# OmarZOS/deep-learning-at-scale

Hardware: AMD Instinct MI355X
Metric: rows/sec (whole node), LSTM seq64 regression at 1/2/4/8 MI355X; val MSE parity (higher is better)
Workload: dtype bf16; 1 GPU; global_batch=8192, per_gpu_batch=8192, seq_len=64, parallelism=dp1

## Files before the change

deep-learning-at-scale_amd/csrc/binding.cpp:

```cpp
#include <torch/extension.h>
#include <ATen/hip/impl/HIPStreamMasqueradingAsCUDA.h>
#include <ATen/hip/impl/HIPGuardImplMasqueradingAsCUDA.h>

#include <cstdlib>
#include <map>
#include <type_traits>
#include <mutex>
#include <vector>

#include "kernels.h"

namespace {

using wf::bf16_t;

int diag_env(const char* name, int dflt) {
  if (wf::dbg_mask() != ~0) return dflt;
  const char* v = std::getenv(name);
  return v != nullptr ? std::atoi(v) : dflt;
}

bool disable_glds() {
  static const bool off = diag_env("WELLFLOW_NO_GLDS", 0) == 1;
  return off;
}

hipStream_t cur_stream() { return c10::hip::getCurrentHIPStreamMasqueradingAsCUDA().stream(); }

void check_t(const at::Tensor& t, at::ScalarType dt, const char* name) {
  TORCH_CHECK(t.defined(), name, ": undefined tensor");
  TORCH_CHECK(t.is_cuda(), name, ": must be a GPU tensor");
  TORCH_CHECK(t.scalar_type() == dt, name, ": expected dtype ", dt, " got ", t.scalar_type());
  TORCH_CHECK(t.is_contiguous(), name, ": must be contiguous");
  TORCH_CHECK(reinterpret_cast<uintptr_t>(t.data_ptr()) % 16 == 0, name,
              ": data pointer must be 16-byte aligned");
}

void check_extent(const at::Tensor& t, int64_t need, const char* name) {
  TORCH_CHECK(t.numel() >= need, name, ": needs at least ", need, " elements, has ", t.numel());
}

bf16_t* bfp(const at::Tensor& t) { return reinterpret_cast<bf16_t*>(t.data_ptr()); }
float* fp(const at::Tensor& t) { return t.data_ptr<float>(); }

template <class T>
T* opt_ptr(const c10::optional<at::Tensor>& t, at::ScalarType dt, const char* name,
           int64_t need) {
  if (!t.has_value() || !t->defined()) return nullptr;
  check_t(*t, dt, name);
  check_extent(*t, need, name);
  return reinterpret_cast<T*>(t->data_ptr());
}

int64_t operand_extent(bool mn, int64_t rows, int64_t K, int64_t ld) {
  if (rows == 0 || K == 0) return 0;
  return mn ? (K - 1) * ld + rows : (rows - 1) * ld + K;
}

void gemm(const at::Tensor& A, bool a_mn, int64_t lda, const at::Tensor& B, bool b_mn, int64_t ldb,
          int64_t M, int64_t N, int64_t K, int64_t ksplit, c10::optional<at::Tensor> outF,
          c10::optional<at::Tensor> outH, int64_t ldo, c10::optional<at::Tensor> bias,
          c10::optional<at::Tensor> mask, int64_t ldm, double mask_scale,
          c10::optional<at::Tensor> colsum, double alpha, double beta, int64_t act, bool atomic,
          double drop_p, int64_t seed, int64_t big_tile, c10::optional<at::Tensor> seed_dev) {
  TORCH_CHECK(wf::dw_tile_valid(big_tile), "gemm: tile ", big_tile, " does not exist; valid ids are 0 (128x128), ",
              "1 (256x128), 3 (256x192), 4 / 5 (256x192, 5- / 4-slot ring), 7 (best for N)");
  check_t(A, at::kBFloat16, "A");
  check_t(B, at::kBFloat16, "B");
  TORCH_CHECK(M > 0 && N > 0 && K > 0, "gemm: empty problem");
  TORCH_CHECK(lda % 8 == 0 && ldb % 8 == 0, "gemm: lda/ldb must be multiples of 8");
  TORCH_CHECK(a_mn ? (M % 8 == 0) : (K % 8 == 0), "gemm: A contiguous extent must be a multiple of 8");
  TORCH_CHECK(b_mn ? (N % 8 == 0) : (K % 8 == 0), "gemm: B contiguous extent must be a multiple of 8");
  TORCH_CHECK(a_mn ? lda >= M : lda >= K, "gemm: lda too small");
  TORCH_CHECK(b_mn ? ldb >= N : ldb >= K, "gemm: ldb too small");
  check_extent(A, operand_extent(a_mn, M, K, lda), "A");
  check_extent(B, operand_extent(b_mn, N, K, ldb), "B");
  TORCH_CHECK(ldo >= N, "gemm: ldo < N");
  const int64_t out_need = (M - 1) * ldo + N;
  wf::GemmEpilogue e;
  e.outF = opt_ptr<float>(outF, at::kFloat, "outF", out_need);
  e.outH = opt_ptr<bf16_t>(outH, at::kBFloat16, "outH", out_need);
  TORCH_CHECK(e.outF || e.outH, "gemm: need an output");
  TORCH_CHECK(!atomic || (e.outF && !e.outH && beta == 0.0), "gemm: atomic needs outF only, beta 0");
  TORCH_CHECK(beta == 0.0 || e.outF, "gemm: beta needs outF");
  e.ldo = ldo;
  e.bias = opt_ptr<float>(bias, at::kFloat, "bias", N);
  if (mask.has_value() && mask->defined()) TORCH_CHECK(ldm >= N, "gemm: ldm < N");
  e.mask = opt_ptr<bf16_t>(mask, at::kBFloat16, "mask", (M - 1) * ldm + N);
  e.ldm = ldm;
  e.mask_scale = (float)mask_scale;
  e.colsum = opt_ptr<float>(colsum, at::kFloat, "colsum", N);
  e.alpha = (float)alpha;
  e.beta = (float)beta;
  e.act = (int)act;
  e.atomic = atomic ? 1 : 0;
  e.drop_p = (float)drop_p;
  e.seed = (unsigned long long)seed;
  if (seed_dev.has_value() && seed_dev->defined()) {
    TORCH_CHECK(seed_dev->is_cuda() && seed_dev->scalar_type() == at::kLong && seed_dev->numel() >= 1,
                "gemm: seed_dev must be a GPU int64 tensor");
    e.seed_dev = reinterpret_cast<const long long*>(seed_dev->data_ptr<int64_t>());
  }
  e.big_tile = (int)big_tile;
  TORCH_CHECK(ksplit == 1 || atomic, "gemm: split-K needs atomic accumulation");
  e.stage_ok = (e.outH != nullptr && e.outF == nullptr && !atomic && beta == 0.0 && N % 8 == 0 &&
                ldo % 8 == 0 && (e.mask == nullptr || ldm % 8 == 0))
                   ? 1 : 0;
  const int64_t Mc = (M + 127) / 128 * 128, Nc = (N + 127) / 128 * 128;
  int64_t kchunk = (K + std::max<int64_t>(ksplit, 1) - 1) / std::max<int64_t>(ksplit, 1);
  kchunk = (kchunk + 63) / 64 * 64;
  const bool glds_ok = (K % 64 == 0) && (kchunk % 64 == 0) &&
                       A.numel() >= operand_extent(a_mn, Mc, K, lda) + (a_mn ? 0 : 0) &&
                       B.numel() >= operand_extent(b_mn, Nc, K, ldb) &&
                       (a_mn || Mc == M || lda >= K) && (b_mn || Nc == N || ldb >= K);
  const c10::hip::OptionalHIPGuardMasqueradingAsCUDA guard(A.device());
  wf::launch_gemm(bfp(A), lda, a_mn, bfp(B), ldb, b_mn, (int)M, (int)N, (int)K, (int)ksplit, e,
                  cur_stream(), glds_ok && !disable_glds());
}

wf::LstmDims lstm_dims(int64_t B, int64_t T, int64_t F, int64_t KX, int64_t H) {
  TORCH_CHECK(B > 0 && T > 0 && H > 0, "lstm: bad dims");
  TORCH_CHECK(H % 128 == 0, "lstm: hidden size must be a multiple of 128");
  TORCH_CHECK(KX % 64 == 0 && F + 1 <= KX, "lstm: KX must be a multiple of 64 and > F");
  wf::LstmDims d;
  d.B = (int)B; d.T = (int)T; d.F = (int)F; d.KX = (int)KX; d.H = (int)H;
  d.xcd_map = diag_env("WELLFLOW_XCD_MAP", 1) == 0 ? 0 : 1;
  d.nt = diag_env("WELLFLOW_NT", 1) == 0 ? 0 : 1;
  const char* pd = std::getenv("WELLFLOW_PF_DBG");
  d.dbg = (pd != nullptr ? std::atoi(pd) : 0) & wf::dbg_mask();
  const char* sl = std::getenv("WELLFLOW_SPIN_LIMIT");
  d.spin_limit = sl != nullptr ? (unsigned)std::strtoul(sl, nullptr, 10) : 0u;
  const char* ft = std::getenv("WELLFLOW_FORCE_TIMEOUT");
  if (ft != nullptr && ft[0] == '1') d.dbg |= 1 << 21;
  return d;
}

void check_lstm_state(const at::Tensor& XH, const at::Tensor& Cst, const at::Tensor& S,
                      const wf::LstmDims& d) {
  const int64_t KA = d.KX + d.H, G = 4 * d.H;
  const int64_t Bp = (d.B + 15) / 16 * 16;
  check_t(XH, at::kBFloat16, "XH");
  check_t(Cst, at::kBFloat16, "Cst");
  check_t(S, at::kBFloat16, "S");
  check_extent(XH, (int64_t)(d.T + 1) * d.B * KA, "XH");
  check_extent(Cst, (int64_t)(d.T + 1) * Bp * d.H, "Cst");
  check_extent(S, (int64_t)d.T * Bp * G, "S");
}

void lstm_pack_x(const at::Tensor& x, const at::Tensor& XH, int64_t B, int64_t T, int64_t F,
                 int64_t KX, int64_t H, bool full) {
  auto d = lstm_dims(B, T, F, KX, H);
  check_t(x, at::kFloat, "x");
  check_extent(x, B * T * F, "x");
  check_t(XH, at::kBFloat16, "XH");
  check_extent(XH, (T + 1) * B * (KX + H), "XH");
  const c10::hip::OptionalHIPGuardMasqueradingAsCUDA guard(x.device());
  wf::launch_lstm_pack_x(fp(x), bfp(XH), d, cur_stream(), full);
}

void lstm_pack_x_win(const at::Tensor& table, const at::Tensor& starts, const at::Tensor& idx, const at::Tensor& XH,
                     int64_t B, int64_t T, int64_t F, int64_t KX, int64_t H, bool full) {
  auto d = lstm_dims(B, T, F, KX, H);
  check_t(table, at::kFloat, "table");
  TORCH_CHECK(table.dim() == 2 && table.size(1) == F && table.size(0) >= T, "lstm_pack_x_win: table must be [>= T][F]");
  check_t(starts, at::kLong, "starts");
  check_t(idx, at::kLong, "idx");
  check_extent(idx, B, "idx");
  TORCH_CHECK(starts.numel() >= 1, "lstm_pack_x_win: no windows");
  check_t(XH, at::kBFloat16, "XH");
  check_extent(XH, (T + 1) * B * (KX + H), "XH");
  const c10::hip::OptionalHIPGuardMasqueradingAsCUDA guard(table.device());
  wf::launch_lstm_pack_x(fp(table), bfp(XH), d, cur_stream(), full, reinterpret_cast<const long*>(starts.data_ptr<int64_t>()),
                         reinterpret_cast<const long*>(idx.data_ptr<int64_t>()), starts.numel(), table.size(0));
}

void lstm_forward(const at::Tensor& XH, const at::Tensor& Wp, const at::Tensor& Cst,
                  const at::Tensor& S, const at::Tensor& cf32, int64_t B, int64_t T, int64_t F, int64_t KX,
                  int64_t H, int64_t variant) {
  auto d = lstm_dims(B, T, F, KX, H);
  d.fwd_variant = (int)variant;
  check_lstm_state(XH, Cst, S, d);
  check_t(Wp, at::kBFloat16, "Wp");
  check_extent(Wp, 4 * H * (KX + H), "Wp");
  check_t(cf32, at::kFloat, "cf32");
  check_extent(cf32, (B + 15) / 16 * 16 * H, "cf32");
  const c10::hip::OptionalHIPGuardMasqueradingAsCUDA guard(XH.device());
  auto s = cur_stream();
  for (int t = 0; t < d.T; ++t) wf::launch_lstm_fwd_step(t, bfp(XH), bfp(Wp), bfp(Cst), bfp(S), fp(cf32), d, s);
}

void check_sync(const at::Tensor& sync) {
  check_t(sync, at::kInt, "sync");
}

bool persistent_status(int st, const char* what) {
  TORCH_CHECK(st >= 0, what, ": launch failed: ", hipGetErrorString((hipError_t)(-st)));
  return st == 1;
}

bool lstm_forward_persistent(const at::Tensor& XH, const at::Tensor& Wp, const at::Tensor& Cst,
                             const at::Tensor& S, const at::Tensor& sync, int64_t B, int64_t T, int64_t F,
                             int64_t KX, int64_t H) {
  auto d = lstm_dims(B, T, F, KX, H);
  check_lstm_state(XH, Cst, S, d);
  check_t(Wp, at::kBFloat16, "Wp");
  check_extent(Wp, 4 * H * (KX + H), "Wp");
  check_sync(sync);
  const c10::hip::OptionalHIPGuardMasqueradingAsCUDA guard(XH.device());
  return persistent_status(wf::launch_lstm_fwd_persistent(bfp(XH), bfp(Wp), bfp(Cst), bfp(S),
                                                          reinterpret_cast<unsigned*>(sync.data_ptr<int>()),
                                                          sync.numel(), d, cur_stream()),
                           "persistent LSTM forward");
}

void check_lstm_bwd(const at::Tensor& WhhT, const at::Tensor& DG, const at::Tensor& dcarry, const at::Tensor& dy,
                    const at::Tensor& w_out, int64_t B, int64_t T, int64_t H) {
  check_t(WhhT, at::kBFloat16, "WhhT");
  check_extent(WhhT, H * 4 * H, "WhhT");
// ... 1178 lines not shown
```

deep-learning-at-scale_amd/csrc/gemm.hip:

```cpp
#include <cstdlib>

#include "gemm_core.h"
#include "kernels.h"

namespace wf {

__device__ __forceinline__ unsigned long long drop_seed(const GemmEpilogue& e) {
  return e.seed_dev != nullptr ? e.seed ^ ((unsigned long long)e.seed_dev[0] * 0xD1B54A32D192ED03ull) : e.seed;
}

template <int BM, int BN, int LA, int LB, int STAGES, int WM = 2, int WN = 2>
__global__ __launch_bounds__(64 * WM * WN) void gemm_kernel(const bf16_t* __restrict__ A, long lda,
                                                   const bf16_t* __restrict__ B, long ldb,
                                                   int M, int N, int K, int kchunk,
                                                   GemmEpilogue e) {
  using C = GemmCfg<BM, BN, LA, LB, WM, WN>;
  constexpr int LDSB = STAGES * C::STAGE > C::LDS_BYTES ? STAGES * C::STAGE : C::LDS_BYTES;
  __shared__ __attribute__((aligned(16))) char smem[LDSB];
  const int tiles_n = (N + BN - 1) / BN;
  const int tiles = ((M + BM - 1) / BM) * tiles_n;
  const int L = xcd_remap(blockIdx.x, gridDim.x);
  const int split = L / tiles, t = L % tiles;
  const int m0 = (t / tiles_n) * BM, n0 = (t % tiles_n) * BN;
  const int kbeg = split * kchunk;
// ... 23 lines not shown
        *reinterpret_cast<uint4*>(mt + chunk_off(row, c8)) = v;
      }
      __syncthreads();
    }
#pragma unroll
    for (int j = 0; j < C::TN; ++j) {
      const int n = cc.col(j);
      const int col = n - n0;
      const bool nok = n < N;
      const float bn = (e.bias != nullptr && nok) ? e.bias[n] : 0.f;
      float csum = 0.f;
#pragma unroll
      for (int i = 0; i < C::TM; ++i) {
#pragma unroll
        for (int r = 0; r < 4; ++r) {
          const int m = cc.row(i, r);
          const int row = m - m0;
          const int lo = chunk_off(row, col >> 3) + (col & 7);
          float v = e.alpha * acc[i][j][r] + bn;
          if (e.act == 1) v = fmaxf(v, 0.f);
          if (e.drop_p > 0.f)
            v = uniform_hash(drop_seed(e), (unsigned long long)m * N + n) >= e.drop_p
                    ? v * (1.f / (1.f - e.drop_p)) : 0.f;
          if (e.mask != nullptr) v = bf2f(mt[lo]) > 0.f ? v * e.mask_scale : 0.f;
          const bf16_t vb = f2bf(v);
          ot[lo] = vb;
          if (nok && m < M) csum += bf2f(vb);
        }
      }
      if (e.colsum != nullptr) {
        csum += __shfl_xor(csum, 16, 64);
        csum += __shfl_xor(csum, 32, 64);
        if ((threadIdx.x & 63) < 16 && nok) atomicAdd(e.colsum + n, csum);
      }
    }
    __syncthreads();
    for (int q = threadIdx.x; q < BM * CPR; q += C::NT) {
      const int row = q / CPR, c8 = q % CPR;
      const int m = m0 + row, n = n0 + c8 * 8;
      if (m < M && n < N)
        *reinterpret_cast<uint4*>(e.outH + (size_t)m * e.ldo + n) =
            *reinterpret_cast<const uint4*>(ot + chunk_off(row, c8));
    }
    return;
  }

#pragma unroll
  for (int j = 0; j < C::TN; ++j) {
    const int n = cc.col(j);
    const bool nok = n < N;
    const float bn = (e.bias != nullptr && nok) ? e.bias[n] : 0.f;
    float csum = 0.f;
#pragma unroll
    for (int i = 0; i < C::TM; ++i) {
#pragma unroll
      for (int r = 0; r < 4; ++r) {
        const int m = cc.row(i, r);
        if (!nok || m >= M) continue;
        float v = e.alpha * acc[i][j][r];
        const size_t o = (size_t)m * e.ldo + n;
        if (e.atomic) {
          atomicAdd(e.outF + o, v);
          continue;
        }
        if (e.beta != 0.f) v += e.beta * e.outF[o];
        v += bn;
        if (e.act == 1) v = fmaxf(v, 0.f);
        if (e.drop_p > 0.f)
          v = uniform_hash(drop_seed(e), (unsigned long long)m * N + n) >= e.drop_p
                  ? v * (1.f / (1.f - e.drop_p)) : 0.f;
        if (e.mask != nullptr)
          v = bf2f(e.mask[(size_t)m * e.ldm + n]) > 0.f ? v * e.mask_scale : 0.f;
        csum += v;
        if (e.outF != nullptr) e.outF[o] = v;
        if (e.outH != nullptr) e.outH[o] = f2bf(v);
      }
    }
    if (e.colsum != nullptr) {
      csum += __shfl_xor(csum, 16, 64);
      csum += __shfl_xor(csum, 32, 64);
      if ((threadIdx.x & 63) < 16 && nok) atomicAdd(e.colsum + n, csum);
    }
  }
}

template <int BM, int BN, int LA, int LB>
static void launch_cfg(const bf16_t* A, long lda, const bf16_t* B, long ldb, int M, int N, int K,
                       int ksplit, const GemmEpilogue& e, hipStream_t s, bool glds_ok) {
  const int tiles = ((M + BM - 1) / BM) * ((N + BN - 1) / BN);
  if (ksplit < 1) ksplit = 1;
  int kchunk = (K + ksplit - 1) / ksplit;
  kchunk = (kchunk + 63) / 64 * 64;
  if (kchunk < 64) kchunk = 64;
  const int nsplit = (K + kchunk - 1) / kchunk;
  const dim3 grid(tiles * (nsplit > 0 ? nsplit : 1));
  if (glds_ok && K % 64 == 0)
    hipLaunchKernelGGL((gemm_kernel<BM, BN, LA, LB, 3>), grid, dim3(256), 0, s, A, lda, B, ldb, M,
                       N, K, kchunk, e);
  else
    hipLaunchKernelGGL((gemm_kernel<BM, BN, LA, LB, 0>), grid, dim3(256), 0, s, A, lda, B, ldb, M,
                       N, K, kchunk, e);
}


static void launch_dw_big(const bf16_t* A, long lda, const bf16_t* B, long ldb, int M, int N, int K,
                          int ksplit, const GemmEpilogue& e, hipStream_t s) {
  constexpr int BM = 256, BN = 128;
  const int tiles = ((M + BM - 1) / BM) * ((N + BN - 1) / BN);
  int kchunk = ((K + ksplit - 1) / ksplit + 63) / 64 * 64;
  const int nsplit = (K + kchunk - 1) / kchunk;
  hipLaunchKernelGGL((gemm_kernel<BM, BN, MN_CONTIG, MN_CONTIG, 3, 4, 2>), dim3(tiles * nsplit),
                     dim3(512), 0, s, A, lda, B, ldb, M, N, K, kchunk, e);
}

template <int BM, int BN, int STAGES, int WM, int WN, int PRIO = 0>
__global__ __launch_bounds__(64 * WM * WN) void gemm_dw_kernel(const bf16_t* __restrict__ A, long lda,
                                                      const bf16_t* __restrict__ B, long ldb, int N,
                                                      int kchunk, int tiles, float* __restrict__ out,
                                                      long ldo, float alpha) {
  using C = GemmCfg<BM, BN, MN_CONTIG, MN_CONTIG, WM, WN>;
  __shared__ __attribute__((aligned(16))) char smem[STAGES * C::STAGE];
  const int tiles_n = N / BN;
  const int L = xcd_remap(blockIdx.x, gridDim.x);
  const int split = L / tiles, t = L % tiles;
  const int m0 = (t / tiles_n) * BM, n0 = (t % tiles_n) * BN;
  f32x4 acc[C::TM][C::TN];
  gemm_mainloop_glds2<C, STAGES, PRIO>(A, lda, B, ldb, split * kchunk, kchunk / 64, m0, n0, smem, acc);
  const AccCoord<C> cc(m0, n0);
#pragma unroll
  for (int j = 0; j < C::TN; ++j)
#pragma unroll
    for (int i = 0; i < C::TM; ++i)
#pragma unroll
      for (int r = 0; r < 4; ++r)
        atomicAdd(out + (size_t)cc.row(i, r) * ldo + cc.col(j), alpha * acc[i][j][r]);
}

static int equal_ksplit(int K, int ksplit) {
  int nsplit = ksplit;
  while (nsplit > 1 && K % (64 * nsplit) != 0) --nsplit;
  return nsplit;
}

static void launch_dw_192(const bf16_t* A, long lda, const bf16_t* B, long ldb, int M, int N, int K,
                          int ksplit, const GemmEpilogue& e, hipStream_t s) {
  constexpr int BM = 256, BN = 192;
  const int tiles = (M / BM) * (N / BN);
  const int nsplit = equal_ksplit(K, ksplit);
  const int kchunk = K / nsplit;
  hipLaunchKernelGGL((gemm_dw_kernel<BM, BN, 2, 4, 2, 1>), dim3(tiles * nsplit), dim3(512), 0, s, A, lda, B, ldb,
                     N, kchunk, tiles, e.outF, e.ldo, e.alpha);
}

template <int BM, int BN, int NSLOT, int WM, int WN, int PRIO, int BKD = 32>
__global__ __launch_bounds__(64 * WM * WN) void gemm_dw_h_kernel(const bf16_t* __restrict__ A, long lda,
                                                        const bf16_t* __restrict__ B, long ldb, int N,
                                                        int kchunk, int tiles, float* __restrict__ out,
                                                        long ldo, float alpha, float* __restrict__ slab,
                                                        long slab_stride) {
  using C = GemmCfg<BM, BN, MN_CONTIG, MN_CONTIG, WM, WN>;
  constexpr int STAGE = (BM + BN) * BKD * 2;
  __shared__ __attribute__((aligned(16))) char smem[NSLOT * STAGE];
  const int tiles_n = N / BN;
  const int L = xcd_remap(blockIdx.x, gridDim.x);
  const int split = L / tiles, t = L % tiles;
  const int m0 = (t / tiles_n) * BM, n0 = (t % tiles_n) * BN;
  f32x4 acc[C::TM][C::TN];
  gemm_mainloop_glds_h<C, NSLOT, PRIO, BKD>(A, lda, B, ldb, split * kchunk, kchunk / BKD, m0, n0, smem, acc);
  const AccCoord<C> cc(m0, n0);
  if (slab != nullptr) {
    float* o = slab + (size_t)split * slab_stride;
#pragma unroll
    for (int j = 0; j < C::TN; ++j)
#pragma unroll
      for (int i = 0; i < C::TM; ++i)
#pragma unroll
        for (int r = 0; r < 4; ++r) o[(size_t)cc.row(i, r) * ldo + cc.col(j)] = alpha * acc[i][j][r];
    return;
  }
#pragma unroll
  for (int j = 0; j < C::TN; ++j)
#pragma unroll
    for (int i = 0; i < C::TM; ++i)
#pragma unroll
      for (int r = 0; r < 4; ++r)
        atomicAdd(out + (size_t)cc.row(i, r) * ldo + cc.col(j), alpha * acc[i][j][r]);
}

static void launch_dw_192h(const bf16_t* A, long lda, const bf16_t* B, long ldb, int M, int N, int K,
                           int ksplit, int nslot, const GemmEpilogue& e, hipStream_t s) {
  constexpr int BM = 256, BN = 192;
  const int tiles = (M / BM) * (N / BN);
  const int nsplit = equal_ksplit(K, ksplit);
  const int kchunk = K / nsplit;
  const dim3 grid(tiles * nsplit);
  if (nslot == 5)
    hipLaunchKernelGGL((gemm_dw_h_kernel<BM, BN, 5, 4, 2, 1>), grid, dim3(512), 0, s, A, lda, B, ldb, N, kchunk,
                       tiles, e.outF, e.ldo, e.alpha, nullptr, 0L);
  else
    hipLaunchKernelGGL((gemm_dw_h_kernel<BM, BN, 4, 4, 2, 1>), grid, dim3(512), 0, s, A, lda, B, ldb, N, kchunk,
                       tiles, e.outF, e.ldo, e.alpha, nullptr, 0L);
}

__global__ __launch_bounds__(256) void dw_slab_reduce_kernel(float* __restrict__ out, const float* __restrict__ slab,
                                                             int nsplit, long n4) {
  const long i = (long)blockIdx.x * 256 + threadIdx.x;
  if (i >= n4) return;
  const float4* src = reinterpret_cast<const float4*>(slab) + i;
  float4 a = reinterpret_cast<float4*>(out)[i];
  for (int s0 = 0; s0 < nsplit; s0 += 8) {
    float4 v[8];
#pragma unroll
    for (int j = 0; j < 8; ++j) v[j] = s0 + j < nsplit ? src[(size_t)(s0 + j) * n4] : make_float4(0.f, 0.f, 0.f, 0.f);
#pragma unroll
    for (int j = 0; j < 8; ++j) {
      a.x += v[j].x;
      a.y += v[j].y;
      a.z += v[j].z;
      a.w += v[j].w;
    }
  }
  reinterpret_cast<float4*>(out)[i] = a;
}

static void launch_dw_288w(const bf16_t* A, long lda, const bf16_t* B, long ldb, int M, int N, int K,
                           int ksplit, const GemmEpilogue& e, hipStream_t s) {
  constexpr int BM = 256, BN = 288;
  const int tiles = (M / BM) * (N / BN);
  static const int cus = [] {
    int dev = 0, n = 0;
    if (hipGetDevice(&dev) != hipSuccess || hipDeviceGetAttribute(&n, hipDeviceAttributeMultiprocessorCount, dev) != hipSuccess)
      return 256;
    return n;
  }();
  if (ksplit * tiles > cus && cus / tiles >= 1) ksplit = cus / tiles;
  const int nsplit = equal_ksplit(K, ksplit);
  const int kchunk = K / nsplit;
  const long mn = (long)M * N;
  const bool use_slab = e.slab != nullptr && e.ldo == N && nsplit > 1 && (long)nsplit * mn <= e.slab_cap && mn % 4 == 0;
  hipLaunchKernelGGL((gemm_dw_h_kernel<BM, BN, 4, 4, 2, 1, 32>), dim3(tiles * nsplit), dim3(512), 0, s, A, lda, B,
                     ldb, N, kchunk, tiles, e.outF, e.ldo, e.alpha, use_slab ? e.slab : nullptr, use_slab ? mn : 0L);
  if (use_slab) {
    const long n4 = mn / 4;
    hipLaunchKernelGGL(dw_slab_reduce_kernel, dim3((unsigned)((n4 + 255) / 256)), dim3(256), 0, s, e.outF,
                       (const float*)e.slab, nsplit, n4);
  }
}

void launch_gemm(const bf16_t* A, long lda, int a_mn, const bf16_t* B, long ldb, int b_mn, int M,
                 int N, int K, int ksplit, const GemmEpilogue& e, hipStream_t s, bool glds_ok) {
  if (a_mn && b_mn && glds_ok && e.atomic && e.big_tile != kDwGeneric && M % 256 == 0 && K % 64 == 0) {
    const int ks = ksplit < 1 ? 1 : ksplit;
    if (e.big_tile == kDwBest && N % 288 == 0)
      launch_dw_288w(A, lda, B, ldb, M, N, K, ks, e, s);
    else if ((e.big_tile == kDw256x192Ring5 || e.big_tile == kDw256x192Ring4) && N % 192 == 0)
      launch_dw_192h(A, lda, B, ldb, M, N, K, ks, e.big_tile == kDw256x192Ring5 ? 5 : 4, e, s);
    else if (e.big_tile != kDw256x128 && N % 192 == 0)
      launch_dw_192(A, lda, B, ldb, M, N, K, ks, e, s);
    else
      launch_dw_big(A, lda, B, ldb, M, N, K, ks, e, s);
    return;
  }
  if (!a_mn && !b_mn)
    launch_cfg<128, 128, K_CONTIG, K_CONTIG>(A, lda, B, ldb, M, N, K, ksplit, e, s, glds_ok);
  else if (!a_mn && b_mn)
    launch_cfg<128, 128, K_CONTIG, MN_CONTIG>(A, lda, B, ldb, M, N, K, ksplit, e, s, glds_ok);
  else if (a_mn && !b_mn)
    launch_cfg<128, 128, MN_CONTIG, K_CONTIG>(A, lda, B, ldb, M, N, K, ksplit, e, s, glds_ok);
  else
    launch_cfg<128, 128, MN_CONTIG, MN_CONTIG>(A, lda, B, ldb, M, N, K, ksplit, e, s, glds_ok);
}

}
```

deep-learning-at-scale_amd/csrc/gemm_core.h:

```cpp
#pragma once
#include <type_traits>

#include "common.h"

namespace wf {

enum : int { K_CONTIG = 0, MN_CONTIG = 1 };

typedef __attribute__((address_space(3))) bf16x4 lds_bf16x4;

template <int R>
struct MnSwz {
  static constexpr int C = R / 16;
  static constexpr bool POW2 = (C & (C - 1)) == 0;
  static constexpr int RSH = C == 12 ? 1 : (C == 18 ? 2 : 0);
  __host__ __device__ static constexpr int hmask() { return POW2 ? C - 1 : 7; }
  __device__ static __forceinline__ int hk(int k) { return ((k & 3) | ((k >> 1) & 4)) & hmask(); }
  __device__ static __forceinline__ int pos(int j, int h) { return POW2 ? (j ^ h) : (j + (h >> RSH)) % C; }
  __device__ static __forceinline__ int data(int p, int h) { return POW2 ? (p ^ h) : (p + C - (h >> RSH)) % C; }
};

template <int R, int L, int NT_ = 256>
struct OpTile {
  static constexpr int NT = NT_;
// ... 248 lines not shown
      const int hk = (q | ((g & 1) << 2)) & MnSwz<R>::hmask();
#pragma unroll
      for (int i = 0; i < NB; ++i)
        fb[i] = (8 * g + q) * (R * 2) + (MnSwz<R>::pos((rw >> 4) + i, hk) << 5) + p * 8;
    }
  }

  template <int KK, int TOFF>
  __device__ __forceinline__ bf16x8 frag(const char* smem, int i) const {
    if constexpr (L == K_CONTIG) {
      return *reinterpret_cast<const bf16x8*>(smem + fb[KK] + TOFF + i * 16 * 128);
    } else {
      bf16x8 out;
#pragma unroll
      for (int h = 0; h < 2; ++h) {
        const char* a = smem + fb[i] + TOFF + (KK * 32 + 4 * h) * (R * 2);
        bf16x4 v = __builtin_amdgcn_ds_read_tr16_b64_v4i16((lds_bf16x4*)a);
        out[4 * h + 0] = v[0];
        out[4 * h + 1] = v[1];
        out[4 * h + 2] = v[2];
        out[4 * h + 3] = v[3];
      }
      return out;
    }
  }
};

template <class C, int STAGES, int PRIO = 0>
__device__ __forceinline__ void gemm_mainloop_glds2(const bf16_t* __restrict__ A, long lda,
                                                    const bf16_t* __restrict__ B, long ldb, int kbeg,
                                                    int nk, int m0, int n0, char* smem,
                                                    f32x4 (&acc)[C::TM][C::TN]) {
  static_assert(STAGES >= 2 && STAGES <= 6, "2..6 stages");
  using OA = GldsOperand<C::BM, C::LA_, C::NT>;
  using OB = GldsOperand<C::BN, C::LB_, C::NT>;
  constexpr int STAGE = OA::TILE_BYTES + OB::TILE_BYTES;
  constexpr int LPT = OA::Q::PER_WAVE + OB::Q::PER_WAVE;
  const int lane = threadIdx.x & 63;
  const int wid = __builtin_amdgcn_readfirstlane(threadIdx.x >> 6);
  const int wm = wid / C::WN, wn = wid % C::WN;
#pragma unroll
  for (int i = 0; i < C::TM; ++i)
#pragma unroll
    for (int j = 0; j < C::TN; ++j) acc[i][j] = f32x4{0.f, 0.f, 0.f, 0.f};
  if (nk <= 0) return;
  OA oa;
  OB ob;
  oa.init(A, lda, m0, kbeg, wid, lane);
  ob.init(B, ldb, n0, kbeg, wid, lane);
  FragReader<C::BM, C::LA_, C::WTM> fa;
  FragReader<C::BN, C::LB_, C::WTN> fbr;
  fa.init(wm * C::WTM, lane);
  fbr.init(wn * C::WTN, lane);

#pragma unroll
  for (int s = 0; s < STAGES - 1; ++s) {
    if (s < nk) {
      oa.issue(s, smem + s * STAGE, wid);
      ob.issue(s, smem + s * STAGE + OA::TILE_BYTES, wid);
    }
  }

  auto body = [&](int tt, auto uc) {
    constexpr int u = decltype(uc)::value;
    const int ahead = min(nk - 1, tt + STAGES - 2) - tt;
    if constexpr (STAGES >= 5) {
      if (ahead >= STAGES - 2) wait_vmcnt<(STAGES - 2) * LPT>();
      else if (ahead == 3) wait_vmcnt<3 * LPT>();
      else if (ahead == 2) wait_vmcnt<2 * LPT>();
      else if (ahead == 1) wait_vmcnt<LPT>();
      else wait_vmcnt<0>();
    } else if constexpr (STAGES >= 4) {
      if (ahead >= 2) wait_vmcnt<2 * LPT>();
      else if (ahead == 1) wait_vmcnt<LPT>();
      else wait_vmcnt<0>();
    } else if constexpr (STAGES == 3) {
      if (ahead >= 1) wait_vmcnt<LPT>();
      else wait_vmcnt<0>();
    } else {
      wait_vmcnt<0>();
    }
    __builtin_amdgcn_s_barrier();
    asm volatile("" ::: "memory");
    const int tn = tt + STAGES - 1;
    if (tn < nk) {
      constexpr int sn = (u + STAGES - 1) % STAGES;
      oa.issue(tn, smem + sn * STAGE, wid);
      ob.issue(tn, smem + sn * STAGE + OA::TILE_BYTES, wid);
    }
    static_for<0, 2>([&](auto kc) {
      constexpr int KK = decltype(kc)::value;
      bf16x8 a[C::TM], b[C::TN];
#pragma unroll
      for (int i = 0; i < C::TM; ++i) a[i] = fa.template frag<KK, u * STAGE>(smem, i);
#pragma unroll
      for (int j = 0; j < C::TN; ++j) b[j] = fbr.template frag<KK, u * STAGE + OA::TILE_BYTES>(smem, j);
      if constexpr (PRIO == 1) __builtin_amdgcn_s_setprio(1);
#pragma unroll
      for (int i = 0; i < C::TM; ++i)
#pragma unroll
        for (int j = 0; j < C::TN; ++j)
          acc[i][j] = __builtin_amdgcn_mfma_f32_16x16x32_bf16(a[i], b[j], acc[i][j], 0, 0, 0);
      if constexpr (PRIO == 1) __builtin_amdgcn_s_setprio(0);
    });
  };

  int t = 0;
  for (; t + STAGES <= nk; t += STAGES)
    static_for<0, STAGES>([&](auto uc) { body(t + decltype(uc)::value, uc); });
  static_for<0, STAGES>([&](auto uc) {
    if (t + decltype(uc)::value < nk) body(t + decltype(uc)::value, uc);
  });
  __builtin_amdgcn_s_barrier();
  asm volatile("" ::: "memory");
}

template <int R, int L, int NT, int BKD>
struct GldsOpH {
  static_assert(L == MN_CONTIG, "half-step ring: MN-contiguous operands only");
  static constexpr int BYTES = R * BKD * 2;
  static constexpr int PIECES = BYTES / 1024;
  static constexpr int NW = NT / 64;
  static constexpr int MAXPW = (PIECES + NW - 1) / NW;
  static constexpr int REM = PIECES % NW;
  static_assert(BYTES % 1024 == 0 && PIECES >= NW, "tile image must be whole 1-KiB pieces, >= 1 per wave");
  using SW = MnSwz<R>;
  unsigned src[MAXPW];
  __amdgpu_buffer_rsrc_t rsrc;
  int kstep_bytes;

  __device__ __forceinline__ void init(const bf16_t* p, long ld, int row0, int kbeg, int wid, int lane) {
#pragma unroll
    for (int i = 0; i < MAXPW; ++i) {
      const int o = (i * NW + wid) * 1024 + lane * 16;
      const int k = o / (R * 2), b = o % (R * 2);
      const int col = (SW::data(b >> 5, SW::hk(k)) << 4) + (((b >> 4) & 1) << 3);
      src[i] = (unsigned)(((long)k * ld + col) * 2);
    }
    rsrc = __builtin_amdgcn_make_buffer_rsrc(const_cast<bf16_t*>(p + (size_t)kbeg * ld + row0), 0, 0x7FFFFFFF,
                                             0x00020000);
    kstep_bytes = (int)(BKD * ld * 2);
  }
  __device__ __forceinline__ void issue(int step, char* lds_tile, int wid) const {
    const int so = step * kstep_bytes;
#pragma unroll
    for (int i = 0; i < MAXPW; ++i) {
      if (i + 1 < MAXPW || REM == 0 || wid < REM)
        __builtin_amdgcn_raw_ptr_buffer_load_lds(rsrc, (lds_void*)(lds_tile + (i * NW + wid) * 1024), 16, (int)src[i],
                                                 so, 0, 0);
    }
  }
};

template <class C, int NSLOT, int PRIO = 0, int BKD = 32>
__device__ __forceinline__ void gemm_mainloop_glds_h(const bf16_t* __restrict__ A, long lda,
                                                     const bf16_t* __restrict__ B, long ldb, int kbeg,
                                                     int nh, int m0, int n0, char* smem,
                                                     f32x4 (&acc)[C::TM][C::TN]) {
  static_assert(BKD == 32 || BKD == 64, "32- or 64-deep steps");
  static_assert(NSLOT >= 2 && NSLOT <= 6, "2..6 slots");
  using OA = GldsOpH<C::BM, C::LA_, C::NT, BKD>;
  using OB = GldsOpH<C::BN, C::LB_, C::NT, BKD>;
  static_assert(OA::REM == 0 || OB::REM == 0, "at most one operand with an uneven piece split");
  constexpr int STAGE = OA::BYTES + OB::BYTES;
  constexpr int LHI = OA::MAXPW + OB::MAXPW;
  constexpr int LLO = LHI - ((OA::REM | OB::REM) != 0 ? 1 : 0);
  constexpr int NHI = OA::REM ? OA::REM : (OB::REM ? OB::REM : C::NT / 64);
  const int lane = threadIdx.x & 63;
  const int wid = __builtin_amdgcn_readfirstlane(threadIdx.x >> 6);
  const int wm = wid / C::WN, wn = wid % C::WN;
  const bool hi = wid < NHI;
#pragma unroll
  for (int i = 0; i < C::TM; ++i)
#pragma unroll
    for (int j = 0; j < C::TN; ++j) acc[i][j] = f32x4{0.f, 0.f, 0.f, 0.f};
  if (nh <= 0) return;
  OA oa;
  OB ob;
  oa.init(A, lda, m0, kbeg, wid, lane);
  ob.init(B, ldb, n0, kbeg, wid, lane);
  FragReader<C::BM, C::LA_, C::WTM> fa;
  FragReader<C::BN, C::LB_, C::WTN> fbr;
  fa.init(wm * C::WTM, lane);
  fbr.init(wn * C::WTN, lane);

#pragma unroll
  for (int s = 0; s < NSLOT - 1; ++s) {
    if (s < nh) {
      oa.issue(s, smem + s * STAGE, wid);
      ob.issue(s, smem + s * STAGE + OA::BYTES, wid);
    }
  }
  auto body = [&](int tt, auto uc) {
    constexpr int u = decltype(uc)::value;
    const int ahead = min(nh - 1, tt + NSLOT - 2) - tt;
    __builtin_amdgcn_sched_barrier(0);
    static_for<0, NSLOT - 1>([&](auto ac) {
      constexpr int a = NSLOT - 2 - decltype(ac)::value;
      if (ahead == a) {
        if (hi) wait_vmcnt<a * LHI>();
        else wait_vmcnt<a * LLO>();
      }
    });
    __builtin_amdgcn_s_barrier();
    asm volatile("" ::: "memory");
    const int tn = tt + NSLOT - 1;
    if (tn < nh) {
      constexpr int sn = (u + NSLOT - 1) % NSLOT;
      oa.issue(tn, smem + sn * STAGE, wid);
      ob.issue(tn, smem + sn * STAGE + OA::BYTES, wid);
    }
    int so = u * STAGE;
    asm volatile("" : "+v"(so));
    const char* sl = smem + so;
    static_for<0, BKD / 32>([&](auto kc) {
      constexpr int KK = decltype(kc)::value;
      bf16x8 a[C::TM], b[C::TN];
#pragma unroll
      for (int i = 0; i < C::TM; ++i) a[i] = fa.template frag<KK, 0>(sl, i);
#pragma unroll
      for (int j = 0; j < C::TN; ++j) b[j] = fbr.template frag<KK, OA::BYTES>(sl, j);
      if constexpr (PRIO == 1) __builtin_amdgcn_s_setprio(1);
#pragma unroll
      for (int i = 0; i < C::TM; ++i)
#pragma unroll
        for (int j = 0; j < C::TN; ++j)
          acc[i][j] = __builtin_amdgcn_mfma_f32_16x16x32_bf16(a[i], b[j], acc[i][j], 0, 0, 0);
      if constexpr (PRIO == 1) __builtin_amdgcn_s_setprio(0);
    });
  };
  int t = 0;
  for (; t + NSLOT <= nh; t += NSLOT)
    static_for<0, NSLOT>([&](auto uc) { body(t + decltype(uc)::value, uc); });
  static_for<0, NSLOT>([&](auto uc) {
    if (t + decltype(uc)::value < nh) body(t + decltype(uc)::value, uc);
  });
  __builtin_amdgcn_s_barrier();
  asm volatile("" ::: "memory");
}

template <class C>
struct AccCoord {
  int mb, nb;
  __device__ __forceinline__ AccCoord(int m0, int n0) {
    const int wid = threadIdx.x >> 6;
    mb = m0 + (wid / C::WN) * C::WTM;
    nb = n0 + (wid % C::WN) * C::WTN;
  }
  __device__ __forceinline__ int row(int i, int r) const {
    return mb + i * 16 + 4 * ((threadIdx.x & 63) >> 4) + r;
  }
  __device__ __forceinline__ int col(int j) const { return nb + j * 16 + (threadIdx.x & 15); }
};

}
```

deep-learning-at-scale_amd/csrc/kernels.h:

```cpp
#pragma once
#include <hip/hip_runtime.h>
#include <stdint.h>

namespace wf {

typedef unsigned short bf16_t;

enum DwTile : int {
  kDwGeneric = 0,
  kDw256x128 = 1,
  kDw256x192 = 3,
  kDw256x192Ring5 = 4,
  kDw256x192Ring4 = 5,
  kDwBest = 7,
};
inline bool dw_tile_valid(long t) {
  return t == kDwGeneric || t == kDw256x128 || t == kDw256x192 || t == kDw256x192Ring5 || t == kDw256x192Ring4 ||
         t == kDwBest;
}

struct GemmEpilogue {
  float* outF = nullptr;
  bf16_t* outH = nullptr;
  long ldo = 0;
  const float* bias = nullptr;
  const bf16_t* mask = nullptr;
  long ldm = 0;
  float mask_scale = 1.f;
  float* colsum = nullptr;
  float alpha = 1.f, beta = 0.f;
  int act = 0;
  int atomic = 0;
  float drop_p = 0.f;
  unsigned long long seed = 0;
  const long long* seed_dev = nullptr;
  int stage_ok = 0;
  int big_tile = kDwGeneric;
  float* slab = nullptr;
  long slab_cap = 0;
};

void launch_gemm(const bf16_t* A, long lda, int a_mn, const bf16_t* B, long ldb, int b_mn, int M,
                 int N, int K, int ksplit, const GemmEpilogue& e, hipStream_t s,
                 bool glds_ok = false);

struct LstmDims {
  int B, T, F, KX, H;
  int fwd_variant = 0;
  int bwd_variant = 0;
  int xcd_map = 1;
  int nt = 1;
  int dbg = 0;
  int row_off = 0;
  unsigned spin_limit = 0;
};
int dbg_mask();
void launch_lstm_pack_x(const float* x, bf16_t* XH, LstmDims d, hipStream_t s, bool full = true,
                        const long* starts = nullptr, const long* idx = nullptr, long nwin = 0, long nrows = 0);
void launch_lstm_fwd_step(int t, bf16_t* XH, const bf16_t* Wp, bf16_t* Cst, bf16_t* S, float* cf32,
                          LstmDims d, hipStream_t s);
int lstm_persistent_sync_words(int row_blocks);
long lstm_persistent_sync_total(int row_blocks);
int launch_lstm_fwd_persistent(bf16_t* XH, const bf16_t* Wp, bf16_t* Cst, bf16_t* S, unsigned* sync,
                                long sync_words, LstmDims d, hipStream_t s);
int launch_lstm_bwd_persistent(const bf16_t* WhhT, const bf16_t* Cst, const bf16_t* S, bf16_t* DG,
                                const float* dcarry, unsigned* sync, long sync_words, LstmDims d,
                                hipStream_t s);
void launch_lstm_bwd_step(int t, const bf16_t* WhhT, const bf16_t* Cst, const bf16_t* S,
                          bf16_t* DG, float* dcarry, const float* dy, const float* w_out,
                          LstmDims d, hipStream_t s);
void launch_lstm_pack_weights(const float* W, bf16_t* Wp, bf16_t* WhhT, LstmDims d,
                              hipStream_t s);

bool launch_mlp2_fwd(const bf16_t* X, int Fp, const bf16_t* W1, const float* b1, const bf16_t* W2, const float* b2,
                     const float* w3, const float* b3, const float* y, bf16_t* H1, bf16_t* H2, unsigned* M2,
                     float* dw3, float* db3, float* pred, float* dy, float* loss_sum, float dy_scale, int B,
                     const long long* rows, long nrows, hipStream_t s, float* red = nullptr);
bool launch_mlp2_bwd(const bf16_t* H1, const bf16_t* H2, const unsigned* M2, const float* dy, const float* w3, const bf16_t* W2,
                     const bf16_t* X, int Fp, bf16_t* dZ1, bf16_t* dZ2, float* dW1, float* db1, float* db2,
                     float* dw3, float* db3, int B, const bf16_t* W1, const float* b1, const long long* rows,
                     long nrows, hipStream_t s, float* red = nullptr);
bool launch_mlp2_dw2(const bf16_t* dZ2, const bf16_t* X, int Fp, const long long* rows, long nrows, const bf16_t* W1,
                     const float* b1, int B, int nsplit, float* dW2, hipStream_t s, float* red = nullptr);
constexpr int kMlpRedCopies = 64, kMlpRedCopies2 = 4, kMlpRedRow = 9216;
constexpr int kMlpRedLoss = 0, kMlpRedDb3 = 1, kMlpRedDw3 = 2, kMlpRedDb1 = 258, kMlpRedDb2 = 514, kMlpRedDW1 = 770;
constexpr int kMlpRedSlabRows = 256, kMlpRedSlabRow = 256 * 64;
constexpr long kMlpRedSlabOff = (long)kMlpRedCopies * kMlpRedRow + (long)kMlpRedCopies2 * 65536;
constexpr int kMlpRedSlab2Rows = 256;
constexpr long kMlpRedSlab2Off = kMlpRedSlabOff + (long)kMlpRedSlabRows * kMlpRedSlabRow;
constexpr long kMlpRedFloats = kMlpRedSlab2Off + (long)kMlpRedSlab2Rows * 65536;
int mlp2_train_grid(int B);
constexpr int kMlpSmallScratch = 49728 + 65536;
struct MlpSmallArgs {
  const bf16_t* X;
  const float* Y;
  const long long* rows;
  long nrows;
  int Fp, B, K;
  float* p;
  float* m;
  float* v;
  float* step;
  float lr, b1, b2, eps, wd, dy_scale, clip;
  bf16_t* shadow;
  bf16_t* w2t;
  float* loss_acc;
  float* scr;
  unsigned* sync;
  unsigned spin_limit;
  long oW1, ob1, oW2, ob2, ow3, ob3;
  unsigned long long* stamps;
};
bool launch_mlp_small(const MlpSmallArgs& a, hipStream_t s);
constexpr int kCnnSmallScratch = 2 * 28 * 64 * 16 * 2 + 2 * 64 * 16 * 2;
struct CnnSmallArgs {
  const float* X;
  const float* Y;
  const long long* rows;
  long nrows;
  int B, K, O, taps, filters, drop, loss_kind;
  float keep_scale, clip, scale;
  unsigned seed;
  long long* rng;
  float* p;
  float* vel;
  float* step;
  float lr, decay, momentum, gscale;
  int nesterov;
  float* loss_acc;
  float* scr;
  unsigned* sync;
  unsigned spin_limit;
  unsigned long long* stamps;
};
bool launch_cnn_small(const CnnSmallArgs& a, hipStream_t s);
bool mlp_bwd8();
void launch_mlp2_reduce(float* red, int Fp, int B, float* loss_sum, float* db3, float* dw3, float* db1, float* db2,
                        float* dW1, float* dW2, hipStream_t s, int dw2_rows = 0);
bool launch_mlp2_step(const bf16_t* X, int Fp, const bf16_t* W1, const float* b1, const bf16_t* W2, const float* b2,
                      const float* w3, const float* b3, const float* y, float dy_scale, int B, const long long* rows,
                      long nrows, bf16_t* dZ2, float* pred, float* red, bool dz_frag, hipStream_t s,
                      const bf16_t* W2T = nullptr, float clip = 0.f);
int launch_mlp2_dw2f(const bf16_t* dZ2F, const bf16_t* X, int Fp, const long long* rows, long nrows, const bf16_t* W1,
                     const float* b1, int B, int nsplit, float* red, hipStream_t s);

struct CnnDims {
  int L, C, taps, T, Fp, Kc, O;
  float drop_p;
};
bool cnn_fused_supported(const CnnDims& d);
int cnn_fwd_grid(int B);
int cnn_bwd_chunks(int B);
long cnn_part_floats(int B, const CnnDims& d, long* wd, long* wc, long* f);
void launch_cnn_sgd_pack(float* p, float* g, float* vel, long n, float* step, float lr, float decay, float momentum,
                         int nesterov, float gscale, int zero_g, const CnnDims& d, bf16_t* WcA, bf16_t* WdF,
                         bf16_t* WdB, hipStream_t s, const float* clip = nullptr, float clipvalue = 0.f);
void launch_cnn_pack(const float* Wc, const float* Wd, const CnnDims& d, bf16_t* WcA, bf16_t* WdF, bf16_t* WdB,
                     hipStream_t s);
void launch_cnn_forward(const float* x, int B, const CnnDims& d, const bf16_t* WcA, const bf16_t* WdF,
                        const float* bd, const float* y, float* dout, float* pred, float* part, int train,
                        int loss_kind, float clip, float scale, unsigned seed, const long long* rng, hipStream_t s);
void launch_cnn_backward(const float* x, int B, const CnnDims& d, const bf16_t* WcA, const bf16_t* WdB,
                         const float* dout, unsigned seed, const long long* rng, float* part_wd, float* part_wc,
                         hipStream_t s);
void launch_cnn_reduce(const float* part_wd, const float* part_wc, const float* part_f, int B, const CnnDims& d,
                       float* gWc, float* gWd, float* gbd, float* loss_sum, long long* rng, hipStream_t s);

void launch_head_fwd(const bf16_t* Hm, long ldh, int B, int Hd, const float* w, const float* b0,
                     const float* target, float* pred, float* dy, float* loss_sum, float dy_scale,
                     hipStream_t s);
bool launch_head_fwd_bwd(const bf16_t* Hm, long ldh, int B, int Hd, const float* w, const float* b0,
                         const float* target, float* pred, float* dy, float* loss_sum, float dy_scale, float* dw,
// ... 71 lines not shown
```

Before: 2.020 million rows/s.

## Alternate global-to-LDS load issue between wave halves in 288-wide dW GEMM

Adds a SCHED=1 mode to the GLDS mainloop. Each 4-slot pipeline stage is now loaded by only half of the waves, with the two halves alternating by stage parity, instead of every wave issuing a share of every stage. The aim is to spread memory issue and vmcnt waits so each wave spends less time stalled on loads between MFMA bursts, at the cost of more loads per issuing wave. The 288-wide weight-gradient launcher uses this mode by default, and a WF_DIAG-gated tile id keeps the old schedule available for comparison.

```diff
diff --git a/deep-learning-at-scale_amd/csrc/binding.cpp b/deep-learning-at-scale_amd/csrc/binding.cpp
--- a/deep-learning-at-scale_amd/csrc/binding.cpp
+++ b/deep-learning-at-scale_amd/csrc/binding.cpp
@@ -63,7 +63,7 @@
           c10::optional<at::Tensor> mask, int64_t ldm, double mask_scale,
           c10::optional<at::Tensor> colsum, double alpha, double beta, int64_t act, bool atomic,
           double drop_p, int64_t seed, int64_t big_tile, c10::optional<at::Tensor> seed_dev) {
-  TORCH_CHECK(wf::dw_tile_valid(big_tile), "gemm: tile ", big_tile, " does not exist; valid ids are 0 (128x128), ",
+  TORCH_CHECK(wf::dw_tile_valid(big_tile) || wf::dw_tile_diag(big_tile), "gemm: tile ", big_tile, " does not exist; valid ids are 0 (128x128), ",
               "1 (256x128), 3 (256x192), 4 / 5 (256x192, 5- / 4-slot ring), 7 (best for N)");
   check_t(A, at::kBFloat16, "A");
   check_t(B, at::kBFloat16, "B");
diff --git a/deep-learning-at-scale_amd/csrc/gemm.hip b/deep-learning-at-scale_amd/csrc/gemm.hip
--- a/deep-learning-at-scale_amd/csrc/gemm.hip
+++ b/deep-learning-at-scale_amd/csrc/gemm.hip
@@ -199,7 +199,7 @@
                      N, kchunk, tiles, e.outF, e.ldo, e.alpha);
 }
 
-template <int BM, int BN, int NSLOT, int WM, int WN, int PRIO, int BKD = 32>
+template <int BM, int BN, int NSLOT, int WM, int WN, int PRIO, int BKD = 32, int SCHED = 0>
 __global__ __launch_bounds__(64 * WM * WN) void gemm_dw_h_kernel(const bf16_t* __restrict__ A, long lda,
                                                         const bf16_t* __restrict__ B, long ldb, int N,
                                                         int kchunk, int tiles, float* __restrict__ out,
@@ -213,7 +213,7 @@
   const int split = L / tiles, t = L % tiles;
   const int m0 = (t / tiles_n) * BM, n0 = (t % tiles_n) * BN;
   f32x4 acc[C::TM][C::TN];
-  gemm_mainloop_glds_h<C, NSLOT, PRIO, BKD>(A, lda, B, ldb, split * kchunk, kchunk / BKD, m0, n0, smem, acc);
+  gemm_mainloop_glds_h<C, NSLOT, PRIO, BKD, SCHED>(A, lda, B, ldb, split * kchunk, kchunk / BKD, m0, n0, smem, acc);
   const AccCoord<C> cc(m0, n0);
   if (slab != nullptr) {
     float* o = slab + (size_t)split * slab_stride;
@@ -268,6 +268,17 @@
     }
   }
   reinterpret_cast<float4*>(out)[i] = a;
+}
+
+constexpr int kDw288Sched = 1;
+
+bool dw_tile_diag(long t) {
+#ifdef WF_DIAG
+  return t == kDwDiagSched0;
+#else
+  (void)t;
+  return false;
+#endif
 }
 
 static void launch_dw_288w(const bf16_t* A, long lda, const bf16_t* B, long ldb, int M, int N, int K,
@@ -285,8 +296,16 @@
   const int kchunk = K / nsplit;
   const long mn = (long)M * N;
   const bool use_slab = e.slab != nullptr && e.ldo == N && nsplit > 1 && (long)nsplit * mn <= e.slab_cap && mn % 4 == 0;
-  hipLaunchKernelGGL((gemm_dw_h_kernel<BM, BN, 4, 4, 2, 1, 32>), dim3(tiles * nsplit), dim3(512), 0, s, A, lda, B,
-                     ldb, N, kchunk, tiles, e.outF, e.ldo, e.alpha, use_slab ? e.slab : nullptr, use_slab ? mn : 0L);
+  auto go = [&](auto sc) {
+    hipLaunchKernelGGL((gemm_dw_h_kernel<BM, BN, 4, 4, 2, 1, 32, decltype(sc)::value>), dim3(tiles * nsplit),
+                       dim3(512), 0, s, A, lda, B, ldb, N, kchunk, tiles, e.outF, e.ldo, e.alpha,
+                       use_slab ? e.slab : nullptr, use_slab ? mn : 0L);
+  };
+#ifdef WF_DIAG
+  if (e.big_tile == kDwDiagSched0) go(std::integral_constant<int, 0>{});
+  else
+#endif
+    go(std::integral_constant<int, kDw288Sched>{});
   if (use_slab) {
     const long n4 = mn / 4;
     hipLaunchKernelGGL(dw_slab_reduce_kernel, dim3((unsigned)((n4 + 255) / 256)), dim3(256), 0, s, e.outF,
@@ -298,7 +317,7 @@
                  int N, int K, int ksplit, const GemmEpilogue& e, hipStream_t s, bool glds_ok) {
   if (a_mn && b_mn && glds_ok && e.atomic && e.big_tile != kDwGeneric && M % 256 == 0 && K % 64 == 0) {
     const int ks = ksplit < 1 ? 1 : ksplit;
-    if (e.big_tile == kDwBest && N % 288 == 0)
+    if ((e.big_tile == kDwBest || dw_tile_diag(e.big_tile)) && N % 288 == 0)
       launch_dw_288w(A, lda, B, ldb, M, N, K, ks, e, s);
     else if ((e.big_tile == kDw256x192Ring5 || e.big_tile == kDw256x192Ring4) && N % 192 == 0)
       launch_dw_192h(A, lda, B, ldb, M, N, K, ks, e.big_tile == kDw256x192Ring5 ? 5 : 4, e, s);
diff --git a/deep-learning-at-scale_amd/csrc/gemm_core.h b/deep-learning-at-scale_amd/csrc/gemm_core.h
--- a/deep-learning-at-scale_amd/csrc/gemm_core.h
+++ b/deep-learning-at-scale_amd/csrc/gemm_core.h
@@ -424,24 +424,30 @@
   }
 };
 
-template <class C, int NSLOT, int PRIO = 0, int BKD = 32>
+template <class C, int NSLOT, int PRIO = 0, int BKD = 32, int SCHED = 0>
 __device__ __forceinline__ void gemm_mainloop_glds_h(const bf16_t* __restrict__ A, long lda,
                                                      const bf16_t* __restrict__ B, long ldb, int kbeg,
                                                      int nh, int m0, int n0, char* smem,
                                                      f32x4 (&acc)[C::TM][C::TN]) {
   static_assert(BKD == 32 || BKD == 64, "32- or 64-deep steps");
   static_assert(NSLOT >= 2 && NSLOT <= 6, "2..6 slots");
-  using OA = GldsOpH<C::BM, C::LA_, C::NT, BKD>;
-  using OB = GldsOpH<C::BN, C::LB_, C::NT, BKD>;
+  static_assert(SCHED == 0 || (SCHED == 1 && NSLOT == 4), "alternating issuer: 4 slots (issuer = half step & 1)");
+  constexpr bool ALT = SCHED == 1;
+  constexpr int NWV = C::NT / 64;
+  constexpr int NIW = ALT ? NWV / 2 : NWV;
+  using OA = GldsOpH<C::BM, C::LA_, NIW * 64, BKD>;
+  using OB = GldsOpH<C::BN, C::LB_, NIW * 64, BKD>;
   static_assert(OA::REM == 0 || OB::REM == 0, "at most one operand with an uneven piece split");
   constexpr int STAGE = OA::BYTES + OB::BYTES;
   constexpr int LHI = OA::MAXPW + OB::MAXPW;
   constexpr int LLO = LHI - ((OA::REM | OB::REM) != 0 ? 1 : 0);
-  constexpr int NHI = OA::REM ? OA::REM : (OB::REM ? OB::REM : C::NT / 64);
+  constexpr int NHI = OA::REM ? OA::REM : (OB::REM ? OB::REM : NIW);
   const int lane = threadIdx.x & 63;
   const int wid = __builtin_amdgcn_readfirstlane(threadIdx.x >> 6);
   const int wm = wid / C::WN, wn = wid % C::WN;
-  const bool hi = wid < NHI;
+  const int grp = wid / NIW;
+  const int wq = ALT ? wid % NIW : wid;
+  const bool hi = wq < NHI;
 #pragma unroll
   for (int i = 0; i < C::TM; ++i)
 #pragma unroll
@@ -449,8 +455,8 @@
   if (nh <= 0) return;
   OA oa;
   OB ob;
-  oa.init(A, lda, m0, kbeg, wid, lane);
-  ob.init(B, ldb, n0, kbeg, wid, lane);
+  oa.init(A, lda, m0, kbeg, wq, lane);
+  ob.init(B, ldb, n0, kbeg, wq, lane);
   FragReader<C::BM, C::LA_, C::WTM> fa;
   FragReader<C::BN, C::LB_, C::WTN> fbr;
   fa.init(wm * C::WTM, lane);
@@ -458,29 +464,49 @@
 
 #pragma unroll
   for (int s = 0; s < NSLOT - 1; ++s) {
-    if (s < nh) {
-      oa.issue(s, smem + s * STAGE, wid);
-      ob.issue(s, smem + s * STAGE + OA::BYTES, wid);
+    if (s < nh && (!ALT || grp == (s & 1))) {
+      oa.issue(s, smem + s * STAGE, wq);
+      ob.issue(s, smem + s * STAGE + OA::BYTES, wq);
     }
   }
   auto body = [&](int tt, auto uc) {
     constexpr int u = decltype(uc)::value;
     const int ahead = min(nh - 1, tt + NSLOT - 2) - tt;
     __builtin_amdgcn_sched_barrier(0);
-    static_for<0, NSLOT - 1>([&](auto ac) {
-      constexpr int a = NSLOT - 2 - decltype(ac)::value;
-      if (ahead == a) {
-        if (hi) wait_vmcnt<a * LHI>();
-        else wait_vmcnt<a * LLO>();
-      }
-    });
+    if constexpr (ALT) {
+      if (grp == (u & 1)) {
+        if (tt + 2 < nh) {
+          if (hi) wait_vmcnt<LHI>();
+          else wait_vmcnt<LLO>();
+        } else {
+          wait_vmcnt<0>();
+        }
+      }
+    } else {
+      static_for<0, NSLOT - 1>([&](auto ac) {
+        constexpr int a = NSLOT - 2 - decltype(ac)::value;
+        if (ahead == a) {
+          if (hi) wait_vmcnt<a * LHI>();
+          else wait_vmcnt<a * LLO>();
+        }
+      });
+    }
     __builtin_amdgcn_s_barrier();
     asm volatile("" ::: "memory");
     const int tn = tt + NSLOT - 1;
-    if (tn < nh) {
-      constexpr int sn = (u + NSLOT - 1) % NSLOT;
-      oa.issue(tn, smem + sn * STAGE, wid);
-      ob.issue(tn, smem + sn * STAGE + OA::BYTES, wid);
+    constexpr int sn = (u + NSLOT - 1) % NSLOT;
+    if constexpr (ALT) {
+      if (grp == (sn & 1)) {
+        if (tn < nh) {
+          oa.issue(tn, smem + sn * STAGE, wq);
+          ob.issue(tn, smem + sn * STAGE + OA::BYTES, wq);
+        }
+      }
+    } else {
+      if (tn < nh) {
+        oa.issue(tn, smem + sn * STAGE, wq);
+        ob.issue(tn, smem + sn * STAGE + OA::BYTES, wq);
+      }
     }
     int so = u * STAGE;
     asm volatile("" : "+v"(so));
diff --git a/deep-learning-at-scale_amd/csrc/kernels.h b/deep-learning-at-scale_amd/csrc/kernels.h
--- a/deep-learning-at-scale_amd/csrc/kernels.h
+++ b/deep-learning-at-scale_amd/csrc/kernels.h
@@ -13,11 +13,13 @@
   kDw256x192Ring5 = 4,
   kDw256x192Ring4 = 5,
   kDwBest = 7,
+  kDwDiagSched0 = 13,
 };
 inline bool dw_tile_valid(long t) {
   return t == kDwGeneric || t == kDw256x128 || t == kDw256x192 || t == kDw256x192Ring5 || t == kDw256x192Ring4 ||
          t == kDwBest;
 }
+bool dw_tile_diag(long t);
 
 struct GemmEpilogue {
   float* outF = nullptr;
```

New measurement: 2.038 million rows/s, median of 6. No clear change (+0.9%).
